# nirschl-lab/stain2stain

Measured on AMD Instinct MI355X. Metric: paired 256x256 stain tiles/sec (full CFM optimisation step), higher is better.
Workload: dtype bf16

## Files before the change

include/stain2stain_hip.h:

```cpp
#ifndef STAIN2STAIN_HIP_H
#define STAIN2STAIN_HIP_H

#ifdef __cplusplus
extern "C" {
#endif

#define S2S_OK 0
#define S2S_ERR_SHAPE (-1)
#define S2S_ERR_ALIGN (-2)
#define S2S_ERR_DTYPE (-3)
#define S2S_ERR_LAUNCH (-4)
#define S2S_ERR_NULL (-5)

#define S2S_BF16 0
#define S2S_F32 1

int s2s_conv3x3_stat_blocks(int dtype, int B, int H, int W, int Cout);
int s2s_conv3x3_nhwc(int dtype, const void* x0, int ld0, int c0, const void* x1, int ld1, int c1,
                     const void* w_packed, const float* bias, void* y, int ldy, float* stat_part,
                     const float* ep_scale, const float* ep_shift, int relu, int B, int H, int W, int Cout,
                     void* stream);

int s2s_conv3x3_ksplit(int dtype, int B, int H, int W, int Cout, int cin);
int s2s_conv3x3_nhwc_k(int dtype, const void* x0, int ld0, int c0, const void* x1, int ld1, int c1,
                       const void* w_packed, const float* bias, void* y, int ldy, float* stat_part,
                       const float* ep_scale, const float* ep_shift, int relu, float* kwork, int B, int H, int W,
                       int Cout, void* stream);
int s2s_conv3x3_stat_rows(int dtype, int B, int H, int W, int Cout, int c0, int c1, int ld0, int ld1, int has_bias);
int s2s_conv3x3_staged(int dtype, int B, int H, int W, int Cout, int c0, int c1, int ld0, int ld1, int ldy, int stats);
int s2s_conv3x3_family(int dtype, int B, int H, int W, int Cout, int c0, int c1, int ld0, int ld1, int ldy, int has_bias,
                       int has_affine, int stats, int stat_rows, int kwork);
int s2s_conv3x3_plan(int dtype, int B, int H, int W, int Cout, int c0, int c1, int ld0, int ld1, int ldy, int has_bias,
                     int has_affine, int stats, int stat_rows, int kwork, int* out);
int s2s_conv3x3_nhwc_s(int dtype, const void* x0, int ld0, int c0, const void* x1, int ld1, int c1, const void* w_packed,
                       const float* bias, void* y, int ldy, float* stat_part, int stat_rows, const float* ep_scale,
                       const float* ep_shift, int relu, float* kwork, int B, int H, int W, int Cout, void* stream);
int s2s_debug_conv_clock(long* out_host, int n);

int s2s_conv3x3_wgrad_splits(int dtype, int B, int H, int W, int Cin, int Cout);
int s2s_conv3x3_wgrad_plan(int dtype, int B, int H, int W, int Cin, int Cout, int what);
int s2s_conv3x3_wgrad_nhwc(int dtype, const void* dy, int lddy, int Cout, const void* x0, int ld0, int c0,
                           const void* x1, int ld1, int c1, float* part, float* grad_oihw, int accumulate,
                           int B, int H, int W, void* stream);
int s2s_conv3x3_wgrad_phase(int dtype, const void* dy, int lddy, int Cout, const void* x0, int ld0, int c0,
                            const void* x1, int ld1, int c1, float* part, float* grad_oihw, int accumulate,
                            int B, int H, int W, int phases, void* stream);

int s2s_stem_stat_blocks(int B, int H, int W);
int s2s_stem_conv3x3_fwd(int dtype, const float* x_nchw, const float* w_oihw, const float* bias, void* y, int ldy,
                         float* stat_part, int B, int H, int W, int Cin, int Cout, void* stream);
int s2s_stem_wgrad_blocks(int B, int H, int W);
int s2s_stem_conv3x3_wgrad(int dtype, const void* dy, int lddy, const float* x_nchw, float* part, float* dw_oihw,
                           float* dbias, int accumulate, int B, int H, int W, int Cin, int Cout, void* stream);
int s2s_stem_conv3x3_wgrad_ref(int dtype, const void* dy, int lddy, const float* x_nchw, float* part, float* dw_oihw,
                               float* dbias, int accumulate, int B, int H, int W, int Cin, int Cout, void* stream);
int s2s_stem_wgrad_family(int dtype, int lddy, int B, int H, int W, int Cin, int Cout, int reference);
int s2s_head_family(int dtype, int B, int H, int W, int C, int Cout, int forward);
int s2s_head_conv1x1_fwd(int dtype, const void* x, int ldx, const float* w, const float* bias, float* y_nchw, int B,
                         int H, int W, int C, int Cout, void* stream);
int s2s_head_wgrad_blocks(int B, int H, int W);
int s2s_head_conv1x1_bwd(int dtype, const float* dy_nchw, const void* x, int ldx, const float* w, void* dx, int lddx,
                         float* part, float* dw, float* dbias, int accumulate, int B, int H, int W, int C, int Cout,
                         void* stream);

int s2s_head_loss_blocks(int B, int H, int W);
int s2s_head_loss_family(int dtype, int B, int H, int W, int C, int Cout);
int s2s_head_loss_fused(int dtype, const void* x, int ldx, const float* w, const float* bias, const float* u_nchw,
                        float* v_nchw, void* dx, int lddx, float grad_scale, float* part, double* lpart, float* dw,
                        float* dbias, float* loss, int accumulate, int B, int H, int W, int C, int Cout, void* stream);

int s2s_tail_blocks(int B, int H, int W);
int s2s_tail_family(int dtype, int B, int H, int W, int C, int Cout);
int s2s_tail_fwd_loss(int dtype, const void* raw, int ldx, const float* scale, const float* shift, const float* mean,
                      const float* invstd, const float* w, const float* bias, const float* u_nchw, float* v_nchw,
                      float* g_nchw, float grad_scale, float* part, double* lpart, float* bnwork, float* dw,
                      float* dbias, float* loss, float* dgamma, float* dbeta, float* conv_dbias, int accumulate, int B,
                      int H, int W, int C, int Cout, void* stream);
int s2s_tail_bwd_apply(int dtype, const void* raw, int ldx, const float* g_nchw, const float* w, const float* scale,
                       const float* shift, const float* mean, const float* invstd, const float* gamma,
                       const float* bnwork, void* dx, int lddx, int B, int H, int W, int C, int Cout, void* stream);

int s2s_bn_finalize(const float* part, int nblk, int C, long count, const float* gamma, const float* beta,
                    float* running_mean, float* running_var, long* num_batches_tracked, float momentum, float eps,
                    float* mean, float* invstd, float* scale, float* shift, void* stream);
int s2s_bn_finalize_b(const float* part, int nblk, int C, long count, const float* gamma, const float* beta,
                      float* running_mean, float* running_var, long* num_batches_tracked, float momentum, float eps,
                      float* mean, float* invstd, float* scale, float* shift, const float* conv_bias, void* stream);
int s2s_bn_eval_prepare(int C, const float* gamma, const float* beta, const float* running_mean,
                        const float* running_var, float eps, float* scale, float* shift, void* stream);
int s2s_bn_relu_apply(int dtype, const void* x, int ldx, const float* scale, const float* shift, void* y, int ldy,
                      void* pool, int ldp, int B, int H, int W, int C, void* stream);
int s2s_maxpool2(int dtype, const void* x, int ldx, void* pool, int ldp, int B, int H, int W, int C, void* stream);
int s2s_bn_bwd_blocks(int B, int H, int W, int C);
int s2s_bn_relu_bwd(int dtype, const void* g1, int ldg1, const void* gp, int ldgp, const float* scale,
                    const float* shift, const void* x, int ldx, const float* mean, const float* invstd, const float* gamma, float* dgamma,
                    float* dbeta, float* dbias_conv, int accumulate, void* dx, int lddx, float* work, int B, int H,
                    int W, int C, void* stream);
int s2s_bn_partial_sums(const float* part, int nblk, int C, float* sums, void* stream);
int s2s_bn_relu_bwd_phase(int dtype, const void* g1, int ldg1, const void* gp, int ldgp, const float* scale,
                          const float* shift, const void* x, int ldx, const float* mean, const float* invstd,
                          const float* gamma, float* dgamma, float* dbeta, float* dbias_conv, int accumulate, void* dx,
                          int lddx, float* work, int B, int H, int W, int C, long count_total, int phases, void* stream);

int s2s_upsample2x_bilinear_ac_fwd(int dtype, const void* x, int ldx, const float* bias_nc, void* y, int ldy, int B,
                                   int Hin, int Win, int Hout, int Wout, int C, void* stream);
int s2s_upsample2x_bn_relu_fwd(int dtype, const void* x, int ldx, const float* scale, const float* shift,
                               const float* bias_nc, void* y, int ldy, int B, int Hin, int Win, int Hout, int Wout, int C,
                               void* stream);
int s2s_upsample2x_bilinear_ac_fwd_ref(int dtype, const void* x, int ldx, const float* bias_nc, void* y, int ldy, int B,
                                       int Hin, int Win, int Hout, int Wout, int C, void* stream);
int s2s_upsample2x_fwd_family(int ldx, int ldy, int B, int Hin, int Win, int Hout, int Wout, int C, int reference);
int s2s_upsample2x_bilinear_ac_bwd(int dtype, const void* dy, int lddy, void* dx, int lddx, int B, int Hin, int Win,
                                   int Hout, int Wout, int C, void* stream);
int s2s_upsample2x_bilinear_ac_bwd_ref(int dtype, const void* dy, int lddy, void* dx, int lddx, int B, int Hin,
                                       int Win, int Hout, int Wout, int C, void* stream);
int s2s_upsample2x_bwd_family(int lddy, int lddx, int B, int Hin, int Win, int Hout, int Wout, int C, int reference);
int s2s_pixel_sum(int dtype, const void* x, int ldx, float* out_nc, int B, int HW, int C, int accumulate,
                  void* stream);

int s2s_time_embedding(const float* t, float* out, int B, int dim, void* stream);
int s2s_linear_fwd(const float* x, const float* w, const float* bias, float* y, int B, int K, int N, void* stream);
int s2s_linear_bwd(const float* dy, const float* x, const float* w, float* dx, float* dw, float* db, int accumulate,
                   int B, int K, int N, void* stream);
int s2s_silu_fwd(const float* h, float* a, int n, void* stream);
int s2s_silu_bwd(const float* h, const float* da, float* dh, int n, void* stream);
int s2s_cfm_sample(const float* x0, const float* x1, const float* t, const float* eps, float sigma, float* xt,
                   float* ut, int B, long per_sample, void* stream);
int s2s_mse_loss(const float* v, const float* u, float* dv, float grad_scale, float* loss, double* work, long count,
                 void* stream);
// ... 358 lines not shown
```

stain2stain_amd/csrc/conv3x3_wgrad_mfma.hip:

```cpp
#include "common.h"
#include <stdlib.h>
#include <type_traits>

struct WgradArgs {
  const void* dy;
  const void* x0;
  const void* x1;
  float* part;
  int lddy, Cout, ld0, c0, ld1, c1;
  int B, H, W, tilesY, tilesX, ntiles, S;
  int lgc;
  int lgh, lgw;
  int xcd;
};

namespace {

template <typename T> struct WPiece;
template <> struct WPiece<bf16_t> {
  bf16x8 v;
  __device__ __forceinline__ void zero() {
#pragma unroll
    for (int i = 0; i < 8; ++i) v[i] = (bf16_t)0.0f;
  }
// ... 104 lines not shown
        if (ci < a.c0) xreg[i].load(x0 + pix * a.ld0 + ci);
        else if (ci < cin) xreg[i].load(x1 + pix * a.ld1 + (ci - a.c0));
      }
    }
  };
  auto store_tile = [&]() {
#pragma unroll
    for (int i = 0; i < DY_IT; ++i) {
      const int idx = tid + i * 256;
      const int px = idx >> 3, pc = idx & 7;
      if (idx < DY_PIECES)
        dreg[i].to_lds(ldsDY, DY_BYTES, (pc >> 2) * (NPX * 64) + px * 64 + (pc & 3) * 16);
    }
#pragma unroll
    for (int i = 0; i < X_IT; ++i) {
      const int idx = tid + i * 256;
      const int px = idx >> 3, pc = idx & 7;
      if (idx < X_PIECES)
        xreg[i].to_lds(ldsX, X_BYTES, (pc >> 2) * (HALO * 64) + px * 64 + (pc & 3) * 16);
    }
  };

  const char* const Ahi = ldsDY + wco * (NPX * 64) + frag_off;
  const char* const Bhi = ldsX + wci * (HALO * 64) + frag_off;

  int tile = blockIdx.z;
  if (tile < a.ntiles) load_tile(tile);
  for (; tile < a.ntiles; tile += a.S) {
    __syncthreads();
    store_tile();
    __syncthreads();
    if (tile + a.S < a.ntiles) load_tile(tile + a.S);
#pragma unroll
    for (int ks = 0; ks < KSTEPS; ++ks) {
      const int m0 = ks * 16;
      const int py = m0 / TW, px = m0 - py * TW;
      const bf16x8 af = tr_frag(Ahi + m0 * 64, 4 * 64);
      bf16x8 am, al;
      if constexpr (SPLIT) {
        am = tr_frag(Ahi + DY_BYTES + m0 * 64, 4 * 64);
        al = tr_frag(Ahi + 2 * DY_BYTES + m0 * 64, 4 * 64);
      }
#pragma unroll
      for (int tap = 0; tap < 9; ++tap) {
        const int hoff = ((py + tap / 3) * HW_ + px + tap % 3) * 64;
        const bf16x8 bfr = tr_frag(Bhi + hoff, 4 * 64);
        if constexpr (SPLIT) {
          const bf16x8 bm = tr_frag(Bhi + X_BYTES + hoff, 4 * 64);
          const bf16x8 bl = tr_frag(Bhi + 2 * X_BYTES + hoff, 4 * 64);
          acc[tap] = __builtin_amdgcn_mfma_f32_32x32x16_bf16(am, bm, acc[tap], 0, 0, 0);
          acc[tap] = __builtin_amdgcn_mfma_f32_32x32x16_bf16(al, bfr, acc[tap], 0, 0, 0);
          acc[tap] = __builtin_amdgcn_mfma_f32_32x32x16_bf16(af, bl, acc[tap], 0, 0, 0);
          acc[tap] = __builtin_amdgcn_mfma_f32_32x32x16_bf16(am, bfr, acc[tap], 0, 0, 0);
          acc[tap] = __builtin_amdgcn_mfma_f32_32x32x16_bf16(af, bm, acc[tap], 0, 0, 0);
        }
        acc[tap] = __builtin_amdgcn_mfma_f32_32x32x16_bf16(af, bfr, acc[tap], 0, 0, 0);
      }
    }
  }

  const int r = lane & 31, h = lane >> 5;
  const int ci = ci0 + wci * 32 + r;
#pragma unroll
  for (int tap = 0; tap < 9; ++tap) {
#pragma unroll
    for (int j = 0; j < 16; ++j) {
      const int co = co0 + wco * 32 + (j & 3) + 8 * (j >> 2) + 4 * h;
      if (co < a.Cout && ci < cin)
        a.part[(((long)blockIdx.z * 9 + tap) * a.Cout + co) * cin + ci] = acc[tap][j];
    }
  }
}

__device__ __attribute__((aligned(64))) char g_wgrad_zero_page[64];
typedef __attribute__((address_space(3))) void lds_void_t;
typedef __attribute__((address_space(1))) const void gbl_void_t;

__device__ __forceinline__ void dma16_asm(const void* gsrc, unsigned lds_dst) {
  unsigned keep;
  asm volatile("s_mov_b32 %0, m0\n\ts_mov_b32 m0, %2\n\ts_nop 0\n\tglobal_load_lds_dwordx4 %1, off\n\ts_mov_b32 m0, %0"
               : "=&s"(keep) : "v"(gsrc), "s"(lds_dst) : "memory");
}

template <int TH, int TW>
__global__ __launch_bounds__(256, 2) void conv3x3_wgrad_dma_kernel(WgradArgs a) {
  using T = bf16_t;
  constexpr int NW = 4, NT = 9;
  constexpr int NPX = TH * TW;
  constexpr int HW_ = TW + 2, HR = TH + 2, HALO = HR * HW_;
  constexpr int XROWS = (HALO + 31) / 32 * 32;
  constexpr int DY_BYTES = 2 * NPX * 64, X_BYTES = 2 * XROWS * 64;
  constexpr int DYGRP = 2 * NPX / 16, XGRP = 2 * XROWS / 16;
  constexpr int DYG = DYGRP / NW;
  constexpr int XG = XGRP / NW;
  constexpr int BUF = DY_BYTES + X_BYTES;
  constexpr int KSTEPS = NPX / 16;
  static_assert(DYGRP % 4 == 0 && XGRP % 4 == 0, "DMA groups split evenly over 4 waves");

  extern __shared__ __attribute__((aligned(16))) char smem[];
  const T* __restrict__ dy = static_cast<const T*>(a.dy);
  const T* __restrict__ x0 = static_cast<const T*>(a.x0);
  const T* __restrict__ x1 = static_cast<const T*>(a.x1);

  const int tid = threadIdx.x, lane = tid & 63;
  const int wave = __builtin_amdgcn_readfirstlane(tid >> 6);
  const int wco = (wave & 3) >> 1, wci = wave & 1;
  unsigned bx = blockIdx.x, by = blockIdx.y, bz = blockIdx.z;
  if (a.xcd) {
    const unsigned L = bx + gridDim.x * (by + gridDim.y * bz), per = gridDim.x * gridDim.y * gridDim.z / 8;
    unsigned Lq = (L & 7) * per + (L >> 3);
    bx = Lq % gridDim.x; Lq /= gridDim.x;
    by = Lq % gridDim.y; bz = Lq / gridDim.y;
  }
  const int ci0 = bx * 64, co0 = by * 64;
  const int cin = a.c0 + a.c1;
  const int drow = lane >> 2, dslot = lane & 3;
  const int zsplit = (int)bz;

  const int g = lane >> 4, q = (lane & 15) >> 2, p = lane & 3;
  const int frag_off = ((g >> 1) * 8 + q) * 64 + ((g & 1) * 16 + p * 4) * 2;

  f32x16 acc[NT];
#pragma unroll
  for (int t = 0; t < NT; ++t)
#pragma unroll
    for (int j = 0; j < 16; ++j) acc[t][j] = 0.f;

  int dy_off[DYG], dy_py[DYG], dy_px[DYG];
  bool dy_ok[DYG];
#pragma unroll
  for (int j = 0; j < DYG; ++j) {
    const int grp = wave + NW * j;
    const int half = grp / (NPX / 16), px = (grp % (NPX / 16)) * 16 + drow;
    const int co = co0 + half * 32 + dslot * 8;
    dy_py[j] = px / TW; dy_px[j] = px - dy_py[j] * TW;
    dy_ok[j] = co < a.Cout;
    dy_off[j] = (dy_py[j] * a.W + dy_px[j]) * a.lddy + co;
  }
  const T* x_ptr[XG];
  int x_off[XG], x_ld[XG], x_hy[XG], x_hx[XG];
#pragma unroll
  for (int j = 0; j < XG; ++j) {
    const int grp = wave + NW * j;
    const int half = grp / (XROWS / 16), px = (grp % (XROWS / 16)) * 16 + drow;
    const int ci = ci0 + half * 32 + dslot * 8;
    x_hy[j] = px / HW_; x_hx[j] = px - x_hy[j] * HW_;
    x_ptr[j] = nullptr; x_ld[j] = 0;
    if (px < HALO) {
      if (ci < a.c0) { x_ptr[j] = x0 + ci; x_ld[j] = a.ld0; }
      else if (ci < cin) { x_ptr[j] = x1 + (ci - a.c0); x_ld[j] = a.ld1; }
    }
    x_off[j] = ((x_hy[j] - 1) * a.W + (x_hx[j] - 1)) * x_ld[j];
  }

  auto dma_tile = [&](int tile, int buf) {
    int bt = tile;
    const int tx = bt % a.tilesX; bt /= a.tilesX;
    const int ty = bt % a.tilesY;
    const int img = bt / a.tilesY;
    const int y0 = ty * TH, xs = tx * TW;
    const long pixbase = (long)(img * a.H + y0) * a.W + xs;
    const bool interior = y0 >= 1 && y0 + TH + 1 <= a.H && xs >= 1 && xs + TW + 1 <= a.W;
    const unsigned base = (unsigned)(uintptr_t)(__attribute__((address_space(3))) char*)smem + buf * BUF;
    if (interior) {
#pragma unroll
      for (int j = 0; j < DYG; ++j) {
        const void* src = dy_ok[j] ? (const void*)(dy + pixbase * a.lddy + dy_off[j]) : (const void*)g_wgrad_zero_page;
        dma16_asm(src, __builtin_amdgcn_readfirstlane(base + (wave + NW * j) * 1024));
      }
#pragma unroll
      for (int j = 0; j < XG; ++j) {
        const void* src = x_ptr[j] ? (const void*)(x_ptr[j] + pixbase * x_ld[j] + x_off[j]) : (const void*)g_wgrad_zero_page;
        dma16_asm(src, __builtin_amdgcn_readfirstlane(base + DY_BYTES + (wave + NW * j) * 1024));
      }
    } else {
#pragma unroll
      for (int j = 0; j < DYG; ++j) {
        const int gy = y0 + dy_py[j], gx = xs + dy_px[j];
        const void* src = g_wgrad_zero_page;
        if (gy < a.H && gx < a.W && dy_ok[j]) src = dy + pixbase * a.lddy + dy_off[j];
        dma16_asm(src, __builtin_amdgcn_readfirstlane(base + (wave + NW * j) * 1024));
      }
#pragma unroll
      for (int j = 0; j < XG; ++j) {
        const int gy = y0 - 1 + x_hy[j], gx = xs - 1 + x_hx[j];
        const void* src = g_wgrad_zero_page;
        if (x_ptr[j] && gy >= 0 && gy < a.H && gx >= 0 && gx < a.W) src = x_ptr[j] + pixbase * x_ld[j] + x_off[j];
        dma16_asm(src, __builtin_amdgcn_readfirstlane(base + DY_BYTES + (wave + NW * j) * 1024));
      }
    }
  };

  int tile = zsplit;
  int buf = 0;
  if (tile < a.ntiles) dma_tile(tile, 0);
  asm volatile("s_waitcnt vmcnt(0)" ::: "memory");
  __builtin_amdgcn_s_barrier();
  for (; tile < a.ntiles; tile += a.S) {
    if (tile + a.S < a.ntiles) dma_tile(tile + a.S, buf ^ 1);
    const char* const Ahi = smem + buf * BUF + wco * (NPX * 64) + frag_off;
    const char* const Bhi = smem + buf * BUF + DY_BYTES + wci * (XROWS * 64) + frag_off;
#pragma unroll
    for (int ks = 0; ks < KSTEPS; ++ks) {
      const int m0 = ks * 16;
      const int py = m0 / TW, px = m0 - py * TW;
      const bf16x8 af = tr_frag(Ahi + m0 * 64, 4 * 64);
#pragma unroll
      for (int t = 0; t < NT; ++t) {
        const int hoff = ((py + t / 3) * HW_ + px + t % 3) * 64;
        const bf16x8 bfr = tr_frag(Bhi + hoff, 4 * 64);
        acc[t] = __builtin_amdgcn_mfma_f32_32x32x16_bf16(af, bfr, acc[t], 0, 0, 0);
      }
    }
    __builtin_amdgcn_sched_barrier(0);
    asm volatile("s_waitcnt vmcnt(0)" ::: "memory");
    __builtin_amdgcn_s_barrier();
    buf ^= 1;
  }

  const int r = lane & 31, h = lane >> 5;
  const int ci = ci0 + wci * 32 + r;
#pragma unroll
  for (int t = 0; t < NT; ++t) {
#pragma unroll
    for (int j = 0; j < 16; ++j) {
      const int co = co0 + wco * 32 + (j & 3) + 8 * (j >> 2) + 4 * h;
      if (co < a.Cout && ci < cin)
        a.part[(((long)zsplit * 9 + t) * a.Cout + co) * cin + ci] = acc[t][j];
    }
  }
}

template <int ZG>
__global__ __launch_bounds__(64 * ZG) void wgrad_reduce_kernel(const float* __restrict__ part, float* __restrict__ grad, int S, int Cout,
                                    int Cin, int accumulate) {
  __shared__ float tile[ZG][9][65];
  const long n = (long)Cout * Cin;
  const int il = threadIdx.x & 63, zg = threadIdx.x >> 6;
  const long i = (long)blockIdx.x * 64 + il;
  float s[9];
#pragma unroll
  for (int t = 0; t < 9; ++t) s[t] = 0.f;
  if (i < n) {
    for (int z = zg; z < S; z += ZG)
#pragma unroll
      for (int t = 0; t < 9; ++t) s[t] += part[((long)z * 9 + t) * n + i];
  }
#pragma unroll
  for (int t = 0; t < 9; ++t) tile[zg][t][il] = s[t];
  __syncthreads();
  const long base = (long)blockIdx.x * 64 * 9;
  for (int k = threadIdx.x; k < 576; k += 64 * ZG) {
    const long o = base + k;
    if (o < n * 9) {
      const int t = k % 9, j = k / 9;
      float v = 0.f;
#pragma unroll
      for (int g = 0; g < ZG; g += 4) v += (tile[g][t][j] + tile[g + 1][t][j]) + (tile[g + 2][t][j] + tile[g + 3][t][j]);
      grad[o] = accumulate ? grad[o] + v : v;
    }
  }
}

template <typename T, int TH, int TW>
int launch_wgrad(WgradArgs& a, hipStream_t s) {
  constexpr int NIMG = std::is_same<T, float>::value ? 3 : 1;
  constexpr int lds = NIMG * (2 * TH * TW * 64 + 2 * (TH + 2) * (TW + 2) * 64);
  a.tilesY = cdiv(a.H, TH);
  a.tilesX = cdiv(a.W, TW);
  a.ntiles = a.B * a.tilesY * a.tilesX;
  if (a.S > a.ntiles) return S2S_ERR_SHAPE;
  auto kern = conv3x3_wgrad_kernel<T, TH, TW>;
  static unsigned long long attr_devs = 0;
  if (int rc = s2s_allow_dyn_lds(reinterpret_cast<const void*>(kern), lds, &attr_devs)) return rc;
  dim3 grid(cdiv(a.c0 + a.c1, 64), cdiv(a.Cout, 64), a.S);
  hipLaunchKernelGGL(kern, grid, dim3(256), lds, s, a);
  S2S_LAUNCH_CHECK();
  return S2S_OK;
}

template <int TH, int TW>
int launch_wgrad_dma(WgradArgs& a, hipStream_t s) {
  constexpr int XROWS = ((TH + 2) * (TW + 2) + 31) / 32 * 32;
  constexpr int lds = 2 * (2 * TH * TW * 64 + 2 * XROWS * 64);
  a.tilesY = cdiv(a.H, TH);
  a.tilesX = cdiv(a.W, TW);
  a.ntiles = a.B * a.tilesY * a.tilesX;
  if (a.S > a.ntiles) return S2S_ERR_SHAPE;
  auto kern = conv3x3_wgrad_dma_kernel<TH, TW>;
  static unsigned long long attr_devs = 0;
  if (int rc = s2s_allow_dyn_lds(reinterpret_cast<const void*>(kern), lds, &attr_devs)) return rc;
  dim3 grid(cdiv(a.c0 + a.c1, 64), cdiv(a.Cout, 64), a.S);
  hipLaunchKernelGGL(kern, grid, dim3(256), lds, s, a);
  S2S_LAUNCH_CHECK();
  return S2S_OK;
}

template <int TH, int TW, bool S2D = false>
__global__ __launch_bounds__(256, 2) void conv2x2_wgrad_dma_kernel(WgradArgs a) {
  using T = bf16_t;
  constexpr int NT = 4;
  constexpr int NPX = TH * TW;
  constexpr int HW_ = TW + 1, HR = TH + 1, HALO = HR * HW_;
  constexpr int XROWS = (HALO + 31) / 32 * 32;
  constexpr int DY_BYTES = 2 * NPX * 64, X_BYTES = 2 * XROWS * 64;
  constexpr int DYG = 2 * NPX / 16 / 4;
  constexpr int XG = 2 * XROWS / 16 / 4;
  constexpr int BUF = DY_BYTES + X_BYTES;
  constexpr int KSTEPS = NPX / 16;
  static_assert((2 * NPX / 16) % 4 == 0 && (2 * XROWS / 16) % 4 == 0, "DMA groups split evenly over 4 waves");

  extern __shared__ __attribute__((aligned(16))) char smem[];
  const T* __restrict__ dy = static_cast<const T*>(a.dy);
  const T* __restrict__ x0 = static_cast<const T*>(a.x0);

  const int tid = threadIdx.x, lane = tid & 63;
  const int wave = __builtin_amdgcn_readfirstlane(tid >> 6);
  const int wco = wave >> 1, wci = wave & 1;
  const int ci0 = blockIdx.x * 64, co0 = blockIdx.y * 64;
  const int cin = a.c0;
  const int Hi = a.H + 1, Wi = a.W + 1;
  const int drow = lane >> 2, dslot = lane & 3;
  const int zsplit = (int)blockIdx.z;

  const int g = lane >> 4, q = (lane & 15) >> 2, p = lane & 3;
  const int frag_off = ((g >> 1) * 8 + q) * 64 + ((g & 1) * 16 + p * 4) * 2;

  f32x16 acc[NT];
#pragma unroll
  for (int t = 0; t < NT; ++t)
#pragma unroll
    for (int j = 0; j < 16; ++j) acc[t][j] = 0.f;

  int dy_off[DYG], dy_py[DYG], dy_px[DYG];
  bool dy_ok[DYG];
#pragma unroll
  for (int j = 0; j < DYG; ++j) {
    const int grp = wave + 4 * j;
    const int half = grp / (NPX / 16), px = (grp % (NPX / 16)) * 16 + drow;
    const int co = co0 + half * 32 + dslot * 8;
    dy_py[j] = px / TW; dy_px[j] = px - dy_py[j] * TW;
    dy_ok[j] = co < a.Cout;
    dy_off[j] = (dy_py[j] * a.W + dy_px[j]) * a.lddy + co;
  }
  const T* x_ptr[XG];
  int x_off[XG], x_hy[XG], x_hx[XG];
#pragma unroll
  for (int j = 0; j < XG; ++j) {
    const int grp = wave + 4 * j;
    const int half = grp / (XROWS / 16), px = (grp % (XROWS / 16)) * 16 + drow;
    const int ci = ci0 + half * 32 + dslot * 8;
    x_hy[j] = px / HW_; x_hx[j] = px - x_hy[j] * HW_;
    if (S2D) {
      const int rs = ci >> a.lgc;
      x_ptr[j] = (px < HALO && ci < cin) ? x0 + (ci & ((1 << a.lgc) - 1)) : nullptr;
      x_hy[j] = 2 * x_hy[j] + (rs >> 1) - 1;
      x_hx[j] = 2 * x_hx[j] + (rs & 1) - 1;
      x_off[j] = 0;
    } else {
      x_ptr[j] = (px < HALO && ci < cin) ? x0 + ci : nullptr;
      x_off[j] = (x_hy[j] * Wi + x_hx[j]) * a.ld0;
    }
  }

  auto dma_tile = [&](int tile, int buf) {
    int bt = tile;
    const int tx = bt % a.tilesX; bt /= a.tilesX;
    const int ty = bt % a.tilesY;
    const int img = bt / a.tilesY;
    const int y0 = ty * TH, xs = tx * TW;
    const long pixbase = (long)(img * a.H + y0) * a.W + xs;
    const long xbase = (long)(img * Hi + y0) * Wi + xs;
// ... 562 lines not shown
  }
}

__global__ __launch_bounds__(256) void split_sum_kernel(const float* __restrict__ part, float* __restrict__ out, int S, long n,
                                                        int accumulate) {
  const long i = (long)blockIdx.x * 256 + threadIdx.x;
  if (i >= n) return;
  float s0 = 0.f, s1 = 0.f;
  int z = 0;
  for (; z + 1 < S; z += 2) { s0 += part[(long)z * n + i]; s1 += part[(long)(z + 1) * n + i]; }
  if (z < S) s0 += part[(long)z * n + i];
  const float v = s0 + s1;
  out[i] = accumulate ? out[i] + v : v;
}

int p2p_wgrad_target() {
  static const int t = [] { const char* e = getenv("S2S_P2P_WGRAD_BLOCKS"); const int v = e ? atoi(e) : 0; return v > 0 ? v : 256; }();
  return t;
}

int conv2x2_wgrad_splits(int B, int H, int W, int Cin, int Cout) {
  const int nt = B * cdiv(H, 8) * cdiv(W, 16);
  const int mn = cdiv(Cin, 64) * cdiv(Cout, 64);
  int s = p2p_wgrad_target() / mn;
  if (s > 256) s = 256;
  if (s > nt) s = nt;
  if (s < 1) s = 1;
  return s;
}

int wgrad_ntiles(int B, int H, int W) { return B * cdiv(H, 8) * cdiv(W, 16); }

}

extern "C" int s2s_conv3x3_wgrad_splits(int dtype, int B, int H, int W, int Cin, int Cout) {
  if (B <= 0 || H <= 0 || W <= 0 || Cin <= 0 || Cout <= 0) return S2S_ERR_SHAPE;
  const int nt = wgrad_ntiles(B, H, W);
  const int mn = cdiv(Cin, 64) * cdiv(Cout, 64);
  static const int target_env = [] { const char* e = getenv("S2S_WGRAD_BLOCKS"); return e ? atoi(e) : 0; }();
  const int target = target_env ? target_env : 256;
  const int cap = mn == 1 ? 512 : 320;
  int s = target / mn;
  if (target_env == 0 && s >= 1 && (long)s * mn < (long)target * 7 / 8 && (long)(s + 1) * mn <= 2L * target) s += 1;
  if (s > cap) s = cap;
  if (s > nt) s = nt;
  if (s < 1) s = 1;
  return s;
}

namespace {
struct Wgrad3x3Plan {
  int splits, tiles;
  int xcd;
  int fold;
  int kernel;
};
int conv3x3_wgrad_plan(int dtype, int B, int H, int W, int Cin, int Cout, Wgrad3x3Plan& p) {
  const int s = s2s_conv3x3_wgrad_splits(dtype, B, H, W, Cin, Cout);
  if (s < 0) return s;
  if (dtype != S2S_BF16 && dtype != S2S_F32) return S2S_ERR_DTYPE;
  p.splits = s;
  p.tiles = wgrad_ntiles(B, H, W);
  p.kernel = dtype == S2S_BF16 ? 0 : 1;
  static const int xcd_aware = [] { const char* e = getenv("S2S_WGRAD_XCD"); return e ? atoi(e) : 1; }();
  p.xcd = p.kernel == 0 && xcd_aware && ((long)cdiv(Cin, 64) * cdiv(Cout, 64) * s) % 8 == 0;
  p.fold = ((long)Cout * Cin <= 32768 && s >= 32) ? 16 : 4;
  return S2S_OK;
}
}

extern "C" int s2s_conv3x3_wgrad_plan(int dtype, int B, int H, int W, int Cin, int Cout, int what) {
  Wgrad3x3Plan p{};
  if (int rc = conv3x3_wgrad_plan(dtype, B, H, W, Cin, Cout, p)) return rc;
  switch (what) {
    case 0: return p.splits;
    case 1: return p.tiles;
    case 2: return p.xcd;
    case 3: return p.fold;
    case 4: return p.kernel;
    default: return S2S_ERR_SHAPE;
  }
}

extern "C" int s2s_conv3x3_wgrad_phase(int dtype, const void* dy, int lddy, int Cout, const void* x0, int ld0, int c0,
                                       const void* x1, int ld1, int c1, float* part, float* grad_oihw,
                                       int accumulate, int B, int H, int W, int phases, void* stream) {
  if (!dy || !x0 || !part || !grad_oihw) return S2S_ERR_NULL;
  if (phases < 1 || phases > 3) return S2S_ERR_SHAPE;
  if (B <= 0 || H <= 0 || W <= 0 || Cout <= 0 || c0 <= 0 || c1 < 0) return S2S_ERR_SHAPE;
  if ((Cout % 8) || (c0 % 8) || (c1 % 8) || (lddy % 8) || (ld0 % 8) || (ld1 % 8) || (c1 > 0 && !x1)) return S2S_ERR_SHAPE;
  if (((uintptr_t)dy & 15) || ((uintptr_t)x0 & 15) || ((uintptr_t)x1 & 15)) return S2S_ERR_ALIGN;
  WgradArgs a{};
  a.dy = dy; a.x0 = x0; a.x1 = x1; a.part = part;
  a.lddy = lddy; a.Cout = Cout; a.ld0 = ld0; a.c0 = c0; a.ld1 = ld1; a.c1 = c1;
  a.B = B; a.H = H; a.W = W; a.lgc = 0; a.lgh = a.lgw = 0;
  Wgrad3x3Plan plan{};
  if (int prc = conv3x3_wgrad_plan(dtype, B, H, W, c0 + c1, Cout, plan)) return prc;
  a.S = plan.splits;
  a.xcd = plan.xcd;
  hipStream_t s = static_cast<hipStream_t>(stream);
  int rc = S2S_OK;
  if (!(phases & 1)) { if (a.S > plan.tiles) return S2S_ERR_SHAPE; }
  else if (plan.kernel == 0) rc = launch_wgrad_dma<8, 16>(a, s);
  else rc = launch_wgrad<float, 8, 16>(a, s);
  if (rc != S2S_OK || !(phases & 2)) return rc;
  const long n = (long)Cout * (c0 + c1);
  if (plan.fold == 16)
    hipLaunchKernelGGL(wgrad_reduce_kernel<16>, dim3((unsigned)((n + 63) / 64)), dim3(1024), 0, s, part, grad_oihw,
                       a.S, Cout, c0 + c1, accumulate);
  else
    hipLaunchKernelGGL(wgrad_reduce_kernel<4>, dim3((unsigned)((n + 63) / 64)), dim3(256), 0, s, part, grad_oihw,
                       a.S, Cout, c0 + c1, accumulate);
  S2S_LAUNCH_CHECK();
  return S2S_OK;
}

extern "C" int s2s_conv3x3_wgrad_nhwc(int dtype, const void* dy, int lddy, int Cout, const void* x0, int ld0, int c0,
                                      const void* x1, int ld1, int c1, float* part, float* grad_oihw,
                                      int accumulate, int B, int H, int W, void* stream) {
  return s2s_conv3x3_wgrad_phase(dtype, dy, lddy, Cout, x0, ld0, c0, x1, ld1, c1, part, grad_oihw, accumulate, B, H, W, 3,
                                 stream);
}

extern "C" int s2s_conv2x2_wgrad_splits(int B, int H, int W, int Cin, int Cout) {
  if (B <= 0 || H <= 0 || W <= 0 || Cin <= 0 || Cout <= 0) return S2S_ERR_SHAPE;
  return conv2x2_wgrad_splits(B, H, W, Cin, Cout);
}

extern "C" int s2s_conv2x2_wgrad_nhwc(int dtype, const void* dy, int lddy, int Cout, const void* x, int ldx, int cin,
                                      float* part, float* grad2, int accumulate, int B, int H, int W, void* stream) {
  if (!dy || !x || !part || !grad2) return S2S_ERR_NULL;
  if (dtype != S2S_BF16) return S2S_ERR_DTYPE;
  if (B <= 0 || H <= 0 || W <= 0 || Cout <= 0 || cin <= 0) return S2S_ERR_SHAPE;
  if ((Cout % 8) || (cin % 8) || (lddy % 8) || (ldx % 8)) return S2S_ERR_SHAPE;
  if (((uintptr_t)dy & 15) || ((uintptr_t)x & 15)) return S2S_ERR_ALIGN;
  if ((long)B * (H + 1) * (W + 1) >= (1L << 31)) return S2S_ERR_SHAPE;
  WgradArgs a{};
  a.dy = dy; a.x0 = x; a.x1 = nullptr; a.part = part;
  a.lddy = lddy; a.Cout = Cout; a.ld0 = ldx; a.c0 = cin; a.ld1 = 8; a.c1 = 0;
  a.B = B; a.H = H; a.W = W; a.lgc = 0; a.lgh = a.lgw = 0;
  a.S = conv2x2_wgrad_splits(B, H, W, cin, Cout);
  a.tilesY = cdiv(H, 8); a.tilesX = cdiv(W, 16);
  a.ntiles = B * a.tilesY * a.tilesX;
  hipStream_t s = static_cast<hipStream_t>(stream);
  constexpr int TH = 8, TW = 16;
  constexpr int XROWS = ((TH + 1) * (TW + 1) + 31) / 32 * 32;
  constexpr int lds = 2 * (2 * TH * TW * 64 + 2 * XROWS * 64);
  auto kern = conv2x2_wgrad_dma_kernel<TH, TW>;
  static unsigned long long attr_devs = 0;
  if (int rc = s2s_allow_dyn_lds(reinterpret_cast<const void*>(kern), lds, &attr_devs)) return rc;
  dim3 grid(cdiv(cin, 64), cdiv(Cout, 64), a.S);
  hipLaunchKernelGGL(kern, grid, dim3(256), lds, s, a);
  const long n = 4L * Cout * cin;
  hipLaunchKernelGGL(split_sum_kernel, dim3((unsigned)((n + 255) / 256)), dim3(256), 0, s, part, grad2, a.S, n,
                     accumulate);
  S2S_LAUNCH_CHECK();
  return S2S_OK;
}

extern "C" int s2s_conv4x4s1_wgrad_splits(int B, int H, int W, int Cin, int Cout) {
  if (B <= 0 || H <= 0 || W <= 0 || Cin <= 0 || Cout <= 0) return S2S_ERR_SHAPE;
  const int nt = B * cdiv(H, 8) * cdiv(W, 16);
  const int mn = cdiv(Cin, 64) * cdiv(Cout, 64) * 4;
  static const int t1 = [] { const char* e = getenv("S2S_P2P_WGRAD_S1_BLOCKS"); const int v = e ? atoi(e) : 0; return v > 0 ? v : 384; }();
  int s = t1 / mn;
  if (s > 128) s = 128;
  if (s > nt) s = nt;
  if (s < 1) s = 1;
  return s;
}

extern "C" int s2s_conv4x4s1_wgrad_nhwc(int dtype, const void* dy, int lddy, int Cout, const void* x, int ldx, int cin,
                                        float* part, float* grad16, int accumulate, int B, int H, int W,
                                        void* stream) {
  if (!dy || !x || !part || !grad16) return S2S_ERR_NULL;
  if (dtype != S2S_BF16) return S2S_ERR_DTYPE;
  if (B <= 0 || H <= 0 || W <= 0 || Cout <= 0 || cin <= 0) return S2S_ERR_SHAPE;
  if ((Cout % 8) || (cin % 8) || (lddy % 8) || (ldx % 8)) return S2S_ERR_SHAPE;
  if (((uintptr_t)dy & 15) || ((uintptr_t)x & 15)) return S2S_ERR_ALIGN;
  if ((long)B * (H + 1) * (W + 1) >= (1L << 31)) return S2S_ERR_SHAPE;
  WgradArgs a{};
  a.dy = dy; a.x0 = x; a.x1 = nullptr; a.part = part;
  a.lddy = lddy; a.Cout = Cout; a.ld0 = ldx; a.c0 = cin; a.ld1 = 8; a.c1 = 0;
  a.B = B; a.H = H; a.W = W; a.lgc = 0; a.lgh = a.lgw = 0;
  a.S = s2s_conv4x4s1_wgrad_splits(B, H, W, cin, Cout);
  a.tilesY = cdiv(H, 8); a.tilesX = cdiv(W, 16);
  a.ntiles = B * a.tilesY * a.tilesX;
  hipStream_t s = static_cast<hipStream_t>(stream);
  constexpr int TH = 8, TW = 16, KS = 4;
  constexpr int XROWS = (TH * (TW + KS - 1) + 31) / 32 * 32;
  constexpr int lds = 2 * (2 * TH * TW * 64 + 2 * XROWS * 64);
  auto kern = convkxk_wgrad_rows_kernel<TH, TW, KS, 1>;
  static unsigned long long attr_devs = 0;
  if (int rc = s2s_allow_dyn_lds(reinterpret_cast<const void*>(kern), lds, &attr_devs)) return rc;
  dim3 grid(cdiv(cin, 64), cdiv(Cout, 64), a.S * KS);
  hipLaunchKernelGGL(kern, grid, dim3(256), lds, s, a);
  const long n = 16L * Cout * cin;
// ... 120 lines not shown
```

stain2stain_amd/ops.py:

```python
from __future__ import annotations

import contextlib
import ctypes
import os
import sys
from typing import Optional, Tuple

import torch

from . import _native
from ._regionio import gpu_rows

BF16, F32 = 0, 1


def _dt(t: torch.Tensor) -> int:
    if t.dtype == torch.bfloat16:
        return BF16
    if t.dtype == torch.float32:
        return F32
    raise RuntimeError(f"stain2stain_amd: unsupported activation dtype {t.dtype}")


_raw_stream = getattr(torch._C, "_cuda_getCurrentRawStream", None)
# ... 194 lines not shown

def _timed(name: str, work_fn=None):
    def deco(fn):
        def wrapped(*args, **kwargs):
            if _PROFILE is None or (_PROFILE_ONLY is not None and name not in _PROFILE_ONLY):
                return fn(*args, **kwargs)
            e0 = _timing_event()
            e1 = _timing_event()
            e0.record()
            out = fn(*args, **kwargs)
            e1.record()
            _PROFILE.append((name + ("@" + PROFILE_TAG if PROFILE_TAG else ""), work_fn(*args, **kwargs) if work_fn else 0.0, e0, e1))
            return out
        wrapped.__name__ = fn.__name__
        wrapped.__doc__ = fn.__doc__
        return wrapped
    return deco


def _conv_flops(x0, x1, w_packed, bias, cout, **kw) -> float:
    B, H, W, c0 = x0.shape
    cin = c0 + (x1.shape[3] if x1 is not None else 0)
    return 2.0 * B * H * W * cout * 9 * cin


def _wgrad_flops(dy, x0, x1, grad_oihw, accumulate=False) -> float:
    B, H, W, cout = dy.shape
    cin = x0.shape[3] + (x1.shape[3] if x1 is not None else 0)
    return 2.0 * B * H * W * cout * 9 * cin


@_timed("conv3x3_mfma", _conv_flops)
def conv3x3(x0: torch.Tensor, x1: Optional[torch.Tensor], w_packed: torch.Tensor, bias: Optional[torch.Tensor],
            cout: int, *, want_stats: bool = False, scale: Optional[torch.Tensor] = None,
            shift: Optional[torch.Tensor] = None, relu: bool = False, out: Optional[torch.Tensor] = None):
    B, H, W, c0 = x0.shape
    dt = _dt(x0)
    p0, ld0 = _nhwc(x0)
    p1, ld1, c1 = 0, 8, 0
    if x1 is not None:
        if x1.shape[:3] != x0.shape[:3] or x1.dtype != x0.dtype:
            raise RuntimeError("stain2stain_amd: conv3x3 sources disagree in shape/dtype")
        p1, ld1 = _nhwc(x1)
        c1 = x1.shape[3]
    if w_packed.dtype != x0.dtype or w_packed.numel() != _L().s2s_pack_conv3x3_fwd_elems(cout, c0 + c1):
        raise RuntimeError("stain2stain_amd: packed weight does not match (cout, cin, dtype)")
    if out is None:
        out = torch.empty((B, H, W, cout), dtype=x0.dtype, device=x0.device)
    elif out.shape != (B, H, W, cout) or out.dtype != x0.dtype:
        raise RuntimeError("stain2stain_amd: conv3x3 output buffer mismatch")
    py, ldy = _nhwc(out)
    stat, nb = None, 0
    if want_stats:
        nb = _L().s2s_conv3x3_stat_rows(dt, B, H, W, cout, c0, c1, ld0, ld1, int(bias is not None))
        _native.check(min(nb, 0), "conv3x3_stat_rows")
        stat = torch.empty((2, cout, nb), dtype=torch.float32, device=x0.device)
    kwork = None
    if not want_stats:
        nsplit = _L().s2s_conv3x3_ksplit(dt, B, H, W, cout, c0 + c1)
        if nsplit > 1:
            kwork = torch.empty((nsplit, B * H * W, cout), dtype=torch.float32, device=x0.device)
    rc = _L().s2s_conv3x3_nhwc_s(dt, p0, ld0, c0, p1, ld1, c1, _ptr(w_packed), _f32(bias), py, ldy, _f32(stat), nb,
                                 _f32(scale), _f32(shift), int(relu), _f32(kwork), B, H, W, cout, _stream())
    _native.check(rc, "conv3x3")
    return out, stat


CONV3X3_PLAN_FIELDS = ("family", "cfg", "gx", "gy", "grid", "xsp", "xsn", "ksplit", "stat_rows")


def conv3x3_plan(dtype: torch.dtype, B: int, H: int, W: int, c0: int, c1: int, cout: int, *, ld0: Optional[int] = None,
                 ld1: Optional[int] = None, ldy: Optional[int] = None, bias: bool = False, affine: bool = False,
                 stats: bool = False, stat_rows: int = -1, kwork: bool = False) -> dict:
    dt = BF16 if dtype == torch.bfloat16 else F32
    out = (ctypes.c_int * len(CONV3X3_PLAN_FIELDS))()
    rc = _L().s2s_conv3x3_plan(dt, B, H, W, cout, c0, c1, c0 if ld0 is None else ld0, max(c1, 8) if ld1 is None else ld1,
                               cout if ldy is None else ldy, int(bias), int(affine), int(stats),
                               stat_rows if stats else 0, int(kwork), ctypes.cast(out, ctypes.c_void_p))
    _native.check(rc, "conv3x3_plan")
    return dict(zip(CONV3X3_PLAN_FIELDS, (int(v) for v in out)))


def conv3x3_wgrad(dy: torch.Tensor, x0: torch.Tensor, x1: Optional[torch.Tensor], grad_oihw: torch.Tensor,
                  accumulate: bool = False) -> None:
    B, H, W, cout = dy.shape
    c0 = x0.shape[3]
    dt = _dt(dy)
    if x0.dtype != dy.dtype or x0.shape[:3] != dy.shape[:3]:
        raise RuntimeError("stain2stain_amd: conv3x3_wgrad operand mismatch")
    pdy, lddy = _nhwc(dy)
    p0, ld0 = _nhwc(x0)
    p1, ld1, c1 = 0, 8, 0
    if x1 is not None:
        p1, ld1 = _nhwc(x1)
        c1 = x1.shape[3]
    if tuple(grad_oihw.shape) != (cout, c0 + c1, 3, 3):
        raise RuntimeError("stain2stain_amd: conv3x3_wgrad gradient buffer has the wrong shape")
    s = _L().s2s_conv3x3_wgrad_splits(dt, B, H, W, c0 + c1, cout)
    part = _workspace(dy.device, s * 9 * cout * (c0 + c1), "wgrad")
    if _PROFILE is not None and (_PROFILE_ONLY is None or "conv3x3_wgrad_mfma" in _PROFILE_ONLY):
        for name, phase, work in (("conv3x3_wgrad_mfma", 1, _wgrad_flops(dy, x0, x1, grad_oihw)), ("wgrad_fold", 2, 0.0)):
            e0 = _timing_event()
            e1 = _timing_event()
            e0.record()
            rc = _L().s2s_conv3x3_wgrad_phase(dt, pdy, lddy, cout, p0, ld0, c0, p1, ld1, c1, _f32(part), _f32(grad_oihw),
                                              int(accumulate), B, H, W, phase, _stream())
            e1.record()
            _native.check(rc, "conv3x3_wgrad")
            _PROFILE.append((name, work, e0, e1))
        return
    rc = _L().s2s_conv3x3_wgrad_nhwc(dt, pdy, lddy, cout, p0, ld0, c0, p1, ld1, c1, _f32(part), _f32(grad_oihw),
                                     int(accumulate), B, H, W, _stream())
    _native.check(rc, "conv3x3_wgrad")


def conv3x3_wgrad_plan(dtype: torch.dtype, B: int, H: int, W: int, cin: int, cout: int) -> dict:
    dt = BF16 if dtype == torch.bfloat16 else F32
    plan = {}
    for what, name in enumerate(("splits", "tiles", "xcd", "fold", "kernel")):
        plan[name] = _L().s2s_conv3x3_wgrad_plan(dt, B, H, W, cin, cout, what)
        _native.check(min(plan[name], 0), "conv3x3_wgrad_plan")
    return plan


HEAD_FALLBACK_MO4, HEAD_FALLBACK_MO8 = 104, 108


def head_family(dtype: torch.dtype, B: int, H: int, W: int, C: int, cout: int, forward: bool) -> int:
    return _L().s2s_head_family(BF16 if dtype == torch.bfloat16 else F32, B, H, W, C, cout, int(forward))


@_timed("stem_fwd")
def stem_fwd(x_nchw: torch.Tensor, w: torch.Tensor, bias: Optional[torch.Tensor], dtype: torch.dtype,
             want_stats: bool = True):
    B, cin, H, W = x_nchw.shape
    cout = w.shape[0]
    if tuple(w.shape) != (cout, cin, 3, 3):
        raise RuntimeError("stain2stain_amd: stem weight shape")
    y = torch.empty((B, H, W, cout), dtype=dtype, device=x_nchw.device)
    stat = None
    if want_stats:
        stat = torch.empty((2, cout, _L().s2s_stem_stat_blocks(B, H, W)), dtype=torch.float32, device=y.device)
    rc = _L().s2s_stem_conv3x3_fwd(_dt(y), _f32(x_nchw), _f32(w), _f32(bias), y.data_ptr(), cout, _f32(stat), B, H, W,
                                   cin, cout, _stream())
    _native.check(rc, "stem_conv3x3_fwd")
    return y, stat


@_timed("stem_wgrad")
def stem_wgrad(dy: torch.Tensor, x_nchw: torch.Tensor, dw: torch.Tensor, dbias: Optional[torch.Tensor],
               accumulate: bool = False, _reference: bool = False) -> None:
    B, H, W, cout = dy.shape
    cin = x_nchw.shape[1]
    pdy, lddy = _nhwc(dy)
    nb = _L().s2s_stem_wgrad_blocks(B, H, W)
    part = torch.empty(((cin + 2) // 3, 2 * nb, cout, 32), dtype=torch.float32, device=dy.device)
    fn = _L().s2s_stem_conv3x3_wgrad_ref if _reference else _L().s2s_stem_conv3x3_wgrad
    rc = fn(_dt(dy), pdy, lddy, _f32(x_nchw), _f32(part), _f32(dw), _f32(dbias), int(accumulate), B, H, W, cin, cout,
            _stream())
    _native.check(rc, "stem_conv3x3_wgrad")


def stem_wgrad_family(dy: torch.Tensor, x_nchw: torch.Tensor, _reference: bool = False) -> int:
    B, H, W, cout = dy.shape
    rc = _L().s2s_stem_wgrad_family(_dt(dy), _nhwc(dy)[1], B, H, W, x_nchw.shape[1], cout, int(_reference))
    if rc < 0:
        _native.check(rc, "stem_wgrad_family")
    return rc


@_timed("head_fwd")
def head_fwd(x: torch.Tensor, w: torch.Tensor, bias: Optional[torch.Tensor]) -> torch.Tensor:
    B, H, W, C = x.shape
    cout = w.shape[0]
    px, ldx = _nhwc(x)
    y = torch.empty((B, cout, H, W), dtype=torch.float32, device=x.device)
    rc = _L().s2s_head_conv1x1_fwd(_dt(x), px, ldx, _f32(w.reshape(cout, C)), _f32(bias), _f32(y), B, H, W, C, cout,
                                   _stream())
    _native.check(rc, "head_conv1x1_fwd")
    return y

# ... 1481 lines not shown
```

Measured before the change: 2236.

## Add row-ahead wgrad DMA kernel using buffer loads with interleaved prefetch

Adds a ROWAHEAD variant of the MFMA weight-gradient DMA kernel and makes it the default. It walks the tile one halo row per k-step, reusing each x fragment across all three row taps. It issues buffer_load…lds with precomputed per-lane offsets so out-of-bounds lanes need no branching, and interleaves the next tile's LDS DMA and fragment reads with the MFMA chain. The goal is to cut LDS fragment traffic and hide the global-to-LDS transfer behind compute, at the cost of more register pressure, hand-written inline asm and a 2 GB buffer-size limit. The old kernel stays reachable through a reference variant flag.

```diff
diff --git a/include/stain2stain_hip.h b/include/stain2stain_hip.h
--- a/include/stain2stain_hip.h
+++ b/include/stain2stain_hip.h
@@ -45,6 +45,9 @@
 int s2s_conv3x3_wgrad_phase(int dtype, const void* dy, int lddy, int Cout, const void* x0, int ld0, int c0,
                             const void* x1, int ld1, int c1, float* part, float* grad_oihw, int accumulate,
                             int B, int H, int W, int phases, void* stream);
+int s2s_conv3x3_wgrad_phase_variant(int dtype, const void* dy, int lddy, int Cout, const void* x0, int ld0, int c0,
+                                    const void* x1, int ld1, int c1, float* part, float* grad_oihw, int accumulate,
+                                    int B, int H, int W, int phases, int variant, void* stream);
 
 int s2s_stem_stat_blocks(int B, int H, int W);
 int s2s_stem_conv3x3_fwd(int dtype, const float* x_nchw, const float* w_oihw, const float* bias, void* y, int ldy,
diff --git a/stain2stain_amd/csrc/conv3x3_wgrad_mfma.hip b/stain2stain_amd/csrc/conv3x3_wgrad_mfma.hip
--- a/stain2stain_amd/csrc/conv3x3_wgrad_mfma.hip
+++ b/stain2stain_amd/csrc/conv3x3_wgrad_mfma.hip
@@ -210,7 +210,31 @@
                : "=&s"(keep) : "v"(gsrc), "s"(lds_dst) : "memory");
 }
 
-template <int TH, int TW>
+typedef int wg_i32x4 __attribute__((ext_vector_type(4)));
+
+__device__ __forceinline__ wg_i32x4 wg_rsrc(const void* base, long bytes) {
+  const unsigned long long u = (unsigned long long)(uintptr_t)base;
+  return wg_i32x4{(int)(unsigned)u, (int)(unsigned)(u >> 32), (int)bytes, 0x00020000};
+}
+
+__device__ __forceinline__ void dma16_buf(wg_i32x4 rs, unsigned voff, unsigned soff, unsigned lds_dst) {
+  unsigned keep;
+  asm volatile("s_mov_b32 %0, m0\n\ts_mov_b32 m0, %4\n\ts_nop 2\n\tbuffer_load_dwordx4 %1, %2, %3 offen lds\n\ts_mov_b32 m0, %0"
+               : "=&s"(keep) : "v"(voff), "s"(rs), "s"(soff), "s"(lds_dst) : "memory");
+}
+__device__ __forceinline__ void dma16_buf2(wg_i32x4 rs0, unsigned soff0, wg_i32x4 rs1, unsigned soff1, unsigned long long first,
+                                           unsigned voff, unsigned lds_dst) {
+  unsigned keep;
+  unsigned long long save;
+  asm volatile("s_mov_b32 %0, m0\n\ts_mov_b32 m0, %8\n\ts_mov_b64 %1, exec\n\ts_and_b64 exec, %1, %7\n\ts_nop 2\n\t"
+               "buffer_load_dwordx4 %2, %3, %4 offen lds\n\ts_andn2_b64 exec, %1, %7\n\ts_nop 2\n\t"
+               "buffer_load_dwordx4 %2, %5, %6 offen lds\n\ts_mov_b64 exec, %1\n\ts_mov_b32 m0, %0"
+               : "=&s"(keep), "=&s"(save)
+               : "v"(voff), "s"(rs0), "s"(soff0), "s"(rs1), "s"(soff1), "s"(first), "s"(lds_dst)
+               : "memory", "scc");
+}
+
+template <int TH, int TW, bool ROWAHEAD>
 __global__ __launch_bounds__(256, 2) void conv3x3_wgrad_dma_kernel(WgradArgs a) {
   using T = bf16_t;
   constexpr int NW = 4, NT = 9;
@@ -254,6 +278,7 @@
 #pragma unroll
     for (int j = 0; j < 16; ++j) acc[t][j] = 0.f;
 
+  if constexpr (!ROWAHEAD) {
   int dy_off[DYG], dy_py[DYG], dy_px[DYG];
   bool dy_ok[DYG];
 #pragma unroll
@@ -344,6 +369,154 @@
     asm volatile("s_waitcnt vmcnt(0)" ::: "memory");
     __builtin_amdgcn_s_barrier();
     buf ^= 1;
+  }
+  } else {
+  constexpr int NB = TW / 16, NSTEP = HR * NB;
+  constexpr int NDMA = DYG + XG;
+  constexpr int DH = NPX / 16, XH = XROWS / 16;
+  constexpr unsigned OOB = 0xffffff00u;
+  static_assert(TW % 16 == 0, "a k-step is 16 consecutive pixels of one halo row");
+  const int wv = wave & 3;
+  const long npix = (long)a.B * a.H * a.W;
+  const wg_i32x4 rs_dy = wg_rsrc(dy, ((npix - 1) * a.lddy + a.Cout) * 2);
+  const wg_i32x4 rs_x0 = wg_rsrc(x0, ((npix - 1) * a.ld0 + a.c0) * 2);
+  const wg_i32x4 rs_x1 = wg_rsrc(a.c1 ? x1 : x0, a.c1 ? ((npix - 1) * a.ld1 + a.c1) * 2 : 0);
+  const unsigned lds0 = (unsigned)(uintptr_t)(__attribute__((address_space(3))) char*)smem;
+
+  unsigned inv[NDMA];
+#pragma unroll
+  for (int j = 0; j < DYG; ++j) {
+    const int grp = wv + NW * j;
+    const int px = (grp % DH) * 16 + drow, co = co0 + (grp / DH) * 32 + dslot * 8;
+    const int py = px / TW, pxx = px - py * TW;
+    inv[j] = co < a.Cout ? (unsigned)(((py * a.W + pxx) * a.lddy + co) * 2) : OOB;
+  }
+#pragma unroll
+  for (int j = 0; j < XG; ++j) {
+    const int grp = wv + NW * j;
+    const int px = (grp % XH) * 16 + drow, ci = ci0 + (grp / XH) * 32 + dslot * 8;
+    const int hy = px / HW_, hx = px - hy * HW_;
+    unsigned v = OOB;
+    if (px < HALO) {
+      if (ci < a.c0) v = (unsigned)(((hy * a.W + hx) * a.ld0 + ci) * 2);
+      else if (ci < cin) v = (unsigned)(((hy * a.W + hx) * a.ld1 + (ci - a.c0)) * 2);
+    }
+    inv[DYG + j] = v;
+  }
+  bool second[2], mixed = false;
+  unsigned long long first[2];
+#pragma unroll
+  for (int h = 0; h < 2; ++h) {
+    const int c = ci0 + 32 * h;
+    second[h] = c >= a.c0;
+    mixed = mixed || (a.c1 > 0 && c < a.c0 && c + 32 > a.c0);
+    first[h] = __builtin_amdgcn_ballot_w64(c + dslot * 8 < a.c0);
+  }
+
+  unsigned vo[NDMA], so_dy = 0, so_x[2] = {0, 0};
+  auto prep = [&](int tile, bool valid) {
+    int bt = valid ? tile : 0;
+    const int tx = bt % a.tilesX; bt /= a.tilesX;
+    const int ty = bt % a.tilesY;
+    const int img = bt / a.tilesY;
+    const int y0 = ty * TH, xs = tx * TW;
+    const int pixbase = (img * a.H + y0) * a.W + xs;
+    const int xb = pixbase - a.W - 1;
+    const bool interior = valid && y0 >= 1 && y0 + TH + 1 <= a.H && xs >= 1 && xs + TW + 1 <= a.W;
+    so_dy = (unsigned)(pixbase * a.lddy * 2);
+    if (interior) {
+      so_x[0] = (unsigned)(xb * a.ld0 * 2);
+      so_x[1] = (unsigned)(xb * a.ld1 * 2);
+#pragma unroll
+      for (int j = 0; j < NDMA; ++j) vo[j] = inv[j];
+    } else {
+      so_x[0] = 0; so_x[1] = 0;
+      const unsigned b0 = (unsigned)(xb * a.ld0 * 2), b1 = (unsigned)(xb * a.ld1 * 2);
+#pragma unroll
+      for (int j = 0; j < DYG; ++j) {
+        const int px = ((wv + NW * j) % DH) * 16 + drow;
+        const int py = px / TW, pxx = px - py * TW;
+        vo[j] = (valid && y0 + py < a.H && xs + pxx < a.W) ? inv[j] : OOB;
+      }
+#pragma unroll
+      for (int j = 0; j < XG; ++j) {
+        const int grp = wv + NW * j;
+        const int px = (grp % XH) * 16 + drow, ci = ci0 + (grp / XH) * 32 + dslot * 8;
+        const int hy = px / HW_, hx = px - hy * HW_;
+        const int gy = y0 - 1 + hy, gx = xs - 1 + hx;
+        const bool ok = valid && inv[DYG + j] != OOB && gy >= 0 && gy < a.H && gx >= 0 && gx < a.W;
+        vo[DYG + j] = ok ? inv[DYG + j] + (ci < a.c0 ? b0 : b1) : OOB;
+      }
+    }
+  };
+  auto dma = [&](int j, int tobuf, auto mixedc) {
+    const unsigned dstb = lds0 + tobuf * BUF;
+    if (j < DYG) {
+      dma16_buf(rs_dy, vo[j], so_dy, dstb + (wv + NW * j) * 1024);
+    } else {
+      const int grp = wv + NW * (j - DYG), h = grp / XH;
+      const unsigned dst = dstb + DY_BYTES + grp * 1024;
+      if constexpr (decltype(mixedc)::value) {
+        dma16_buf2(rs_x0, so_x[0], rs_x1, so_x[1], h ? first[1] : first[0], vo[j], dst);
+      } else {
+        const bool s = h ? second[1] : second[0];
+        dma16_buf(s ? rs_x1 : rs_x0, vo[j], s ? so_x[1] : so_x[0], dst);
+      }
+    }
+  };
+
+  auto run = [&](auto mixedc) {
+    int tile = zsplit;
+    int buf = 0;
+    prep(tile, true);
+#pragma unroll
+    for (int j = 0; j < NDMA; ++j) dma(j, 0, mixedc);
+    prep(tile + a.S, tile + a.S < a.ntiles);
+    asm volatile("s_waitcnt vmcnt(0)" ::: "memory");
+    __builtin_amdgcn_s_barrier();
+    for (; tile < a.ntiles; tile += a.S) {
+      const char* const Ahi = smem + buf * BUF + wco * (NPX * 64) + frag_off;
+      const char* const Bhi = smem + buf * BUF + DY_BYTES + wci * (XROWS * 64) + frag_off;
+      bf16x8 xf[NSTEP][3], df[TH * NB];
+      auto rd = [&](int k, int it) {
+        const int r = k / NB, b = k - r * NB;
+        if (it < 3) xf[k][it] = tr_frag(Bhi + (r * HW_ + b * 16 + it) * 64, 4 * 64);
+        else df[k] = tr_frag(Ahi + (r * TW + b * 16) * 64, 4 * 64);
+      };
+      rd(0, 0); rd(0, 1); rd(0, 2); rd(0, 3);
+      __builtin_amdgcn_sched_group_barrier(0x100, 8, 0);
+      int m = 0;
+#pragma unroll
+      for (int k = 0; k < NSTEP; ++k) {
+        const int r = k / NB, b = k - r * NB;
+        const int nfr = k + 1 < NSTEP ? ((k + 1) / NB < TH ? 4 : 3) : 0;
+        const int nm = 3 * ((r < 2 ? r : 2) - (r - TH + 1 > 0 ? r - TH + 1 : 0) + 1);
+        int i = 0;
+#pragma unroll
+        for (int ty = 2; ty >= 0; --ty) {
+          if (r - ty < 0 || r - ty >= TH) continue;
+#pragma unroll
+          for (int s = 0; s < 3; ++s) {
+            acc[ty * 3 + s] = __builtin_amdgcn_mfma_f32_32x32x16_bf16(df[(r - ty) * NB + b], xf[k][s], acc[ty * 3 + s], 0, 0, 0);
+            __builtin_amdgcn_sched_group_barrier(0x008, 1, 0);
+#pragma unroll
+            for (int it = i; it < nfr && (it == i || i == nm - 1); ++it) {
+              rd(k + 1, it);
+              __builtin_amdgcn_sched_group_barrier(0x100, 2, 0);
+            }
+            if (m < NDMA) dma(m, buf ^ 1, mixedc);
+            ++m; ++i;
+          }
+        }
+      }
+      __builtin_amdgcn_sched_barrier(0);
+      prep(tile + 2 * a.S, tile + 2 * a.S < a.ntiles);
+      asm volatile("s_waitcnt vmcnt(0)" ::: "memory");
+      __builtin_amdgcn_s_barrier();
+      buf ^= 1;
+    }
+  };
+  if (mixed) run(std::true_type{}); else run(std::false_type{});
   }
 
   const int r = lane & 31, h = lane >> 5;
@@ -407,7 +580,7 @@
   return S2S_OK;
 }
 
-template <int TH, int TW>
+template <int TH, int TW, bool ROWAHEAD>
 int launch_wgrad_dma(WgradArgs& a, hipStream_t s) {
   constexpr int XROWS = ((TH + 2) * (TW + 2) + 31) / 32 * 32;
   constexpr int lds = 2 * (2 * TH * TW * 64 + 2 * XROWS * 64);
@@ -415,7 +588,13 @@
   a.tilesX = cdiv(a.W, TW);
   a.ntiles = a.B * a.tilesY * a.tilesX;
   if (a.S > a.ntiles) return S2S_ERR_SHAPE;
-  auto kern = conv3x3_wgrad_dma_kernel<TH, TW>;
+  if (ROWAHEAD) {
+    const long npix = (long)a.B * a.H * a.W, lim = 0x7fffffffL;
+    if (((npix - 1) * a.lddy + a.Cout) * 2 > lim || ((npix - 1) * a.ld0 + a.c0) * 2 > lim ||
+        (a.c1 && ((npix - 1) * a.ld1 + a.c1) * 2 > lim))
+      return S2S_ERR_SHAPE;
+  }
+  auto kern = conv3x3_wgrad_dma_kernel<TH, TW, ROWAHEAD>;
   static unsigned long long attr_devs = 0;
   if (int rc = s2s_allow_dyn_lds(reinterpret_cast<const void*>(kern), lds, &attr_devs)) return rc;
   dim3 grid(cdiv(a.c0 + a.c1, 64), cdiv(a.Cout, 64), a.S);
@@ -1144,11 +1323,11 @@
   }
 }
 
-extern "C" int s2s_conv3x3_wgrad_phase(int dtype, const void* dy, int lddy, int Cout, const void* x0, int ld0, int c0,
-                                       const void* x1, int ld1, int c1, float* part, float* grad_oihw,
-                                       int accumulate, int B, int H, int W, int phases, void* stream) {
+extern "C" int s2s_conv3x3_wgrad_phase_variant(int dtype, const void* dy, int lddy, int Cout, const void* x0, int ld0, int c0,
+                                               const void* x1, int ld1, int c1, float* part, float* grad_oihw,
+                                               int accumulate, int B, int H, int W, int phases, int variant, void* stream) {
   if (!dy || !x0 || !part || !grad_oihw) return S2S_ERR_NULL;
-  if (phases < 1 || phases > 3) return S2S_ERR_SHAPE;
+  if (phases < 1 || phases > 3 || variant < 0 || variant > 1) return S2S_ERR_SHAPE;
   if (B <= 0 || H <= 0 || W <= 0 || Cout <= 0 || c0 <= 0 || c1 < 0) return S2S_ERR_SHAPE;
   if ((Cout % 8) || (c0 % 8) || (c1 % 8) || (lddy % 8) || (ld0 % 8) || (ld1 % 8) || (c1 > 0 && !x1)) return S2S_ERR_SHAPE;
   if (((uintptr_t)dy & 15) || ((uintptr_t)x0 & 15) || ((uintptr_t)x1 & 15)) return S2S_ERR_ALIGN;
@@ -1163,7 +1342,7 @@
   hipStream_t s = static_cast<hipStream_t>(stream);
   int rc = S2S_OK;
   if (!(phases & 1)) { if (a.S > plan.tiles) return S2S_ERR_SHAPE; }
-  else if (plan.kernel == 0) rc = launch_wgrad_dma<8, 16>(a, s);
+  else if (plan.kernel == 0) rc = variant ? launch_wgrad_dma<8, 16, false>(a, s) : launch_wgrad_dma<8, 16, true>(a, s);
   else rc = launch_wgrad<float, 8, 16>(a, s);
   if (rc != S2S_OK || !(phases & 2)) return rc;
   const long n = (long)Cout * (c0 + c1);
@@ -1175,6 +1354,13 @@
                        a.S, Cout, c0 + c1, accumulate);
   S2S_LAUNCH_CHECK();
   return S2S_OK;
+}
+
+extern "C" int s2s_conv3x3_wgrad_phase(int dtype, const void* dy, int lddy, int Cout, const void* x0, int ld0, int c0,
+                                       const void* x1, int ld1, int c1, float* part, float* grad_oihw,
+                                       int accumulate, int B, int H, int W, int phases, void* stream) {
+  return s2s_conv3x3_wgrad_phase_variant(dtype, dy, lddy, Cout, x0, ld0, c0, x1, ld1, c1, part, grad_oihw, accumulate, B, H, W,
+                                         phases, 0, stream);
 }
 
 extern "C" int s2s_conv3x3_wgrad_nhwc(int dtype, const void* dy, int lddy, int Cout, const void* x0, int ld0, int c0,
diff --git a/stain2stain_amd/ops.py b/stain2stain_amd/ops.py
--- a/stain2stain_amd/ops.py
+++ b/stain2stain_amd/ops.py
@@ -300,7 +300,8 @@
 
 
 def conv3x3_wgrad(dy: torch.Tensor, x0: torch.Tensor, x1: Optional[torch.Tensor], grad_oihw: torch.Tensor,
-                  accumulate: bool = False) -> None:
+                  accumulate: bool = False, _reference: bool = False, _phases: int = 3,
+                  _part: Optional[torch.Tensor] = None) -> None:
     B, H, W, cout = dy.shape
     c0 = x0.shape[3]
     dt = _dt(dy)
@@ -315,6 +316,16 @@
     if tuple(grad_oihw.shape) != (cout, c0 + c1, 3, 3):
         raise RuntimeError("stain2stain_amd: conv3x3_wgrad gradient buffer has the wrong shape")
     s = _L().s2s_conv3x3_wgrad_splits(dt, B, H, W, c0 + c1, cout)
+    if _reference or _phases != 3 or _part is not None:
+        if _part is None:
+            _part = _workspace(dy.device, s * 9 * cout * (c0 + c1), "wgrad")
+        elif _part.dtype != torch.float32 or _part.numel() < s * 9 * cout * (c0 + c1) or not _part.is_contiguous():
+            raise RuntimeError("stain2stain_amd: conv3x3_wgrad slab buffer is too small")
+        rc = _L().s2s_conv3x3_wgrad_phase_variant(dt, pdy, lddy, cout, p0, ld0, c0, p1, ld1, c1, _f32(_part),
+                                                  _f32(grad_oihw), int(accumulate), B, H, W, _phases, int(_reference),
+                                                  _stream())
+        _native.check(rc, "conv3x3_wgrad")
+        return
     part = _workspace(dy.device, s * 9 * cout * (c0 + c1), "wgrad")
     if _PROFILE is not None and (_PROFILE_ONLY is None or "conv3x3_wgrad_mfma" in _PROFILE_ONLY):
         for name, phase, work in (("conv3x3_wgrad_mfma", 1, _wgrad_flops(dy, x0, x1, grad_oihw)), ("wgrad_fold", 2, 0.0)):
```

New measurement: 2266 (median of 6 runs). 1.01x the previous value.
